# Daniel-Starr/pointcloudhookup

Measured on AMD Instinct MI355X. Metric: Mpts/s ground-filter+tower-cluster, 100 M-pt corridor; % HBM roofline on kNN, higher is better.
Workload: dtype f32 (filter) + f64 (distance predicate)

## Files before the change

pointcloudhookup_amd/csrc/pch_dbscan.hip:

```cpp
#include <assert.h>
#include "pch_prims.h"

namespace pch {

constexpr int DB_THREADS = 256;
constexpr int DB_WAVES   = DB_THREADS / 64;
constexpr int DB_ROWS    = 25;
constexpr int INT_BIG    = 0x7fffffff;
constexpr int DB_FEW_QUERIES = 24;
constexpr int DB_AHEAD = 3;
constexpr long long DB_LONG_TOT = 8192;
constexpr int DB_SEGS = 43;

struct DbGrid {
    float   ox, oy, oz;
    double  cell;
    double  inv_cell;
    double  eps2;
    float   eps2_lo, eps2_hi;
    int     bx, by, bz;
    int     mx, my, mz;
    int64_t chunk_size;
    const uint32_t* chunk_bad;
    const uint32_t* chunk_cells;
// ... 760 lines not shown
    int over = 0;
#pragma unroll
    for (int u = 0; u < CC_ITEMS; ++u) {
        const int c = c0 + u;
        v[u] = 0u;
        if (c < nchunks) {
            const int64_t lo = (int64_t)c * chunk_size;
            v[u] = ct_staged_cells(ncell, c, (n - lo) < chunk_size ? (n - lo) : chunk_size);
            over |= ovf[c] != 0u;
        }
        sum += v[u];
    }
    over = __syncthreads_or(over);
    const uint32_t incl = wave_scan_incl(sum);
    if (lane_id() == 63) wsum[wave_id()] = incl;
    __syncthreads();
    uint32_t run = incl - sum, total = 0;
    for (int w = 0; w < CC_THREADS / 64; ++w) { if (w < wave_id()) run += wsum[w]; total += wsum[w]; }
#pragma unroll
    for (int u = 0; u < CC_ITEMS; ++u) {
        if (c0 + u < nchunks) chunk_cells[c0 + u] = run;
        run += v[u];
    }
    if (tid == 0) {
        *route = over ? 1u : 0u;
        if (!over) {
            chunk_cells[nchunks] = total;
            cell_start[total] = (uint32_t)n;
            *ncells = total;
        }
    }
}

__global__ __launch_bounds__(DB_THREADS) void db_celltab_k(
    const uint32_t* __restrict__ route, DbStage st, const uint32_t* __restrict__ ovf,
    const uint32_t* __restrict__ chunk_cells, int64_t n, int64_t chunk_size, uint32_t* __restrict__ cid,
    uint32_t* __restrict__ cell_start, uint64_t* __restrict__ cell_key, int* __restrict__ cell_min,
    uint32_t* __restrict__ bits, uint64_t* __restrict__ keys_out) {
    const int64_t base = (int64_t)blockIdx.x * SCAN_TILE + (int64_t)threadIdx.x * DC_ITEMS;
    const bool fill = *route != 0u;
    if (!fill && base / DC_ITEMS < (n + 31) / 32) bits[base / DC_ITEMS] = 0u;
    if (base >= n) return;
    int64_t c = (uint32_t)base / (uint32_t)chunk_size;
    int64_t lo = c * chunk_size, end = lo + chunk_size < n ? lo + chunk_size : n;
    uint32_t nc = ct_staged_cells(st.ncell, c, end - lo), j = 0;
    for (uint32_t a = 1, b = nc; a < b;) {
        const uint32_t mid = a + (b - a) / 2;
        if (st.start[lo + mid] <= (uint32_t)base) { j = mid; a = mid + 1; } else b = mid;
    }
    int64_t next = j + 1 < nc ? (int64_t)st.start[lo + j + 1] : end;
    uint32_t cell0 = chunk_cells[c];
    bool skip = fill && ovf[c] != 0u;
    uint32_t cc[DC_ITEMS];
#pragma unroll
    for (int u = 0; u < DC_ITEMS; ++u) {
        const int64_t i = base + u;
        cc[u] = 0u;
        if (i >= n) continue;
        bool head = i == base && nc != 0u && (int64_t)st.start[lo + j] == i;
        if (i == end) {
            ++c; lo = end; end = lo + chunk_size < n ? lo + chunk_size : n;
            nc = ct_staged_cells(st.ncell, c, end - lo); j = 0;
            next = 1 < nc ? (int64_t)st.start[lo + 1] : end;
            cell0 = chunk_cells[c];
            skip = fill && ovf[c] != 0u;
            head = nc != 0u;
        } else if (i == next) {
            ++j;
            next = j + 1 < nc ? (int64_t)st.start[lo + j + 1] : end;
            head = true;
        }
        cc[u] = cell0 + j;
        if (fill) {
            if (!skip) keys_out[i] = st.key[lo + j];
        } else if (head) {
            cell_start[cc[u]] = (uint32_t)i;
            cell_key[cc[u]] = st.key[lo + j];
            cell_min[cc[u]] = (int)st.minrow[lo + j];
        }
    }
    if (fill) return;
    if (base + DC_ITEMS <= n) {
        uint4* o = reinterpret_cast<uint4*>(cid + base);
        o[0] = make_uint4(cc[0], cc[1], cc[2], cc[3]);
        o[1] = make_uint4(cc[4], cc[5], cc[6], cc[7]);
    } else {
#pragma unroll
        for (int u = 0; u < DC_ITEMS; ++u)
            if (base + u < n) cid[base + u] = cc[u];
    }
}

struct RowSet {
    int ca[DB_ROWS], cb[DB_ROWS];
};

template <typename K>
__device__ __forceinline__ int db_lower(const K* __restrict__ a, int m, K k) {
    int lo = 0, hi = m;
    while (lo < hi) { const int mid = (lo + hi) >> 1; if (a[mid] < k) lo = mid + 1; else hi = mid; }
    return lo;
}
struct DbRowAt { int xlo, xhi, ny, nz; };
__device__ __forceinline__ bool db_row_at(const DbGrid& g, uint64_t key, int row, DbRowAt& at) {
    const uint64_t cx = key & ((1ull << g.bx) - 1);
    const uint64_t cy = (key >> g.bx) & ((1ull << g.by) - 1);
    const uint64_t cz = (key >> (g.bx + g.by)) & ((1ull << g.bz) - 1);
    at.ny = (int)cy + DB_ROW_DY[row];
    at.nz = (int)cz + DB_ROW_DZ[row];
    at.xlo = (int)cx - 2 < 0 ? 0 : (int)cx - 2;
    at.xhi = (int)cx + 2 > g.mx ? g.mx : (int)cx + 2;
    return at.ny >= 0 && at.ny <= g.my && at.nz >= 0 && at.nz <= g.mz;
}
template <typename K>
__device__ __forceinline__ int2 db_run_in(const K* __restrict__ a, int n, K klo, K khi) {
    int2 v;
    v.x = db_lower(a, n, klo);
    K kk[5];
#pragma unroll
    for (int i = 0; i < 5; ++i) kk[i] = v.x + i < n ? a[v.x + i] : ~K(0);
    int cntx = 0;
#pragma unroll
    for (int i = 0; i < 5; ++i) cntx += kk[i] <= khi ? 1 : 0;
    v.y = v.x + cntx;
    return v;
// ... 11 lines not shown
                      db_pack(g, chunk, (uint64_t)at.nz, (uint64_t)at.ny, (uint64_t)at.xhi));
        v.x += c0;
        v.y += c0;
    }
    return v;
}

__device__ __forceinline__ void db_rows(const DbGrid& g, const uint64_t* __restrict__ cell_key, uint64_t key,
                                        RowSet* __restrict__ rs, const int2* __restrict__ rowtab, int cell) {
    const int l = lane_id();
    if (rowtab) {
        if (l < DB_ROWS) {
            const int2 v = rowtab[(int64_t)cell * DB_ROWS + l];
            rs->ca[l] = v.x;
            rs->cb[l] = v.y;
        }
        __builtin_amdgcn_wave_barrier();
        return;
    }
    if (l < DB_ROWS) {
        const int2 v = db_row_run(g, cell_key, key, l);
        rs->ca[l] = v.x;
        rs->cb[l] = v.y;
    }
    __builtin_amdgcn_wave_barrier();
}

__global__ __launch_bounds__(DB_THREADS) void db_rowtab_k(DbGrid g, const uint64_t* __restrict__ cell_key,
                                                          int m, int2* __restrict__ rowtab) {
    const int c = (blockIdx.x * DB_WAVES + wave_id()) * 2 + (lane_id() >> 5);
    const int l = lane_id() & 31;
    if (c >= m || l >= DB_ROWS) return;
    rowtab[(int64_t)c * DB_ROWS + l] = db_row_run(g, cell_key, cell_key[c], l);
}

template <bool COUNT, int AHEAD>
__device__ __forceinline__ int db_query_sweep(const DbGrid& g, const float4* __restrict__ pts, const float4 qp,
                                              int count, int r, uint32_t j0, const uint32_t* sa, const uint32_t* sb,
                                              unsigned long long& n_useful, unsigned long long& n_slots) {
    const int l = lane_id();
    while (r < DB_SEGS && count < g.min_samples) {
        const uint32_t pb = sb[r];
        if (j0 >= pb) { ++r; if (r < DB_SEGS) j0 = sa[r]; continue; }
        float4 P[AHEAD];
#pragma unroll
        for (int u = 0; u < AHEAD; ++u) {
            const uint32_t j = j0 + 64u * u + l;
            P[u] = pts[j < pb ? j : pb - 1];
        }
#pragma unroll
        for (int u = 0; u < AHEAD; ++u) {
            const uint32_t jb = j0 + 64u * u;
            const bool hit = jb + l < pb && db_within2(qp, P[u], g);
            count += (int)__popcll(__ballot(hit));
            if (COUNT && jb < pb) { n_useful += (pb - jb) < 64u ? (pb - jb) : 64u; n_slots += 64; }
        }
        j0 += 64u * AHEAD;
    }
    return count;
}

__device__ __forceinline__ void db_summary_none(float* __restrict__ cell_box, int* __restrict__ cell_min, int c) {
    const int l = lane_id();
    if (l < 6) cell_box[6 * (int64_t)c + l] = l < 3 ? INFINITY : -INFINITY;
    if (l == 0) cell_min[c] = INT_BIG;
}
// ... 869 lines not shown
    __syncthreads();

    int r = -1;
    if (tid < nc && ncore[tid] != 0) {
        r = uf_find(parent, tid);
        if (r != tid) atomicMin(&cmin[r], cmin[tid]);
    }
    __syncthreads();
    if (tid < nc) {
        const int64_t c = first + tid;
        root[c] = r < 0 ? -1 : first + r;
        comp_min[c] = r == tid ? cmin[tid] : INT_BIG;
        if (r == tid) {
            const uint32_t row = (uint32_t)cmin[tid];
            if ((int64_t)row < n) atomicOr(&flag[row >> 5], 1u << (row & 31u));
        }
    }
}

constexpr int DB_LAB_ROUNDS = 8;
constexpr int DB_LAB_TILE   = DB_THREADS * DB_LAB_ROUNDS;

__device__ __forceinline__ void db_box_flush(uint32_t* __restrict__ acc, int cur, uint32_t (&m)[6]) {
    const int l = lane_id();
    uint32_t v = 0;
#pragma unroll
    for (int a = 0; a < 6; ++a) {
        const uint32_t t = wave_reduce_max(m[a]);
        if (l == a) v = t;
        m[a] = 0u;
    }
    if (cur >= 0 && l < 6 && v) atomicMax(&acc[8 * (int64_t)cur + l], v);
}

__global__ __launch_bounds__(DB_THREADS) void db_label_k(const float4* __restrict__ pts,
                                                         const uint32_t* __restrict__ cid,
                                                         const uint8_t* __restrict__ core_s,
                                                         const int* __restrict__ root,
                                                         const int* __restrict__ comp_min,
                                                         const uint32_t* __restrict__ bits,
                                                         const uint32_t* __restrict__ rank, int64_t n,
                                                         const uint32_t* __restrict__ cell_start,
                                                         int* __restrict__ cell_label,
                                                         int32_t* __restrict__ labels,
                                                         uint8_t* __restrict__ core_out, int64_t chunk_size, int bpc,
                                                         int64_t nchunks, uint32_t* __restrict__ box_acc,
                                                         int32_t box_cap) {
    int64_t lo, hi;
    {
        const int64_t woff = (int64_t)wave_id() * (64 * DB_LAB_ROUNDS);
        if (bpc > 0) {
            const int64_t slot = blockIdx.x >> 3;
            const int64_t c = (slot / bpc) * 8 + (blockIdx.x & 7);
            const int64_t within = (slot % bpc) * DB_LAB_TILE + woff;
            lo = c * chunk_size + within;
            hi = (c < nchunks && within < chunk_size) ? (c + 1) * chunk_size : lo;
        } else {
            lo = (int64_t)blockIdx.x * DB_LAB_TILE + woff;
            hi = n;
        }
        if (hi > n) hi = n;
        if (hi > lo + 64 * DB_LAB_ROUNDS) hi = lo + 64 * DB_LAB_ROUNDS;
    }
    if (lo >= hi) return;
    const int l = lane_id();
    constexpr int R = DB_LAB_ROUNDS;
// ... 8 lines not shown
        c[u] = valid[u] ? cid[i] : 0u;
        p[u] = pts[valid[u] ? i : lo];
        is_core[u] = valid[u] && core_s[i] != 0;
    }
#pragma unroll
    for (int u = 0; u < R; ++u) {
        rt[u] = valid[u] ? root[c[u]] : -1;
        cs[u] = valid[u] ? cell_start[c[u]] : 0xFFFFFFFFu;
    }
#pragma unroll
    for (int u = 0; u < R; ++u) row[u] = rt[u] >= 0 ? (uint32_t)comp_min[rt[u]] : 0u;
#pragma unroll
    for (int u = 0; u < R; ++u) {
        rk[u] = rt[u] >= 0 ? rank[row[u] >> 5] : 0u;
        bw[u] = rt[u] >= 0 ? bits[row[u] >> 5] : 0u;
    }
#pragma unroll
    for (int u = 0; u < R; ++u) {
        const int64_t i = lo + u * 64 + l;
        lab[u] = rt[u] >= 0 ? (int)(rk[u] + (uint32_t)__popc(bw[u] & ((1u << (row[u] & 31u)) - 1u))) : INT_BIG;
        if (valid[u]) {
            const uint32_t o = __float_as_uint(p[u].w);
            labels[o] = is_core[u] ? lab[u] : -1;
            if (core_out) core_out[o] = is_core[u] ? 1 : 0;
            if (cs[u] == (uint32_t)i) cell_label[c[u]] = lab[u];
        }
    }
    if (!box_acc) return;
    int cur = -1;
    uint32_t m[6] = {0u, 0u, 0u, 0u, 0u, 0u};
#pragma unroll
    for (int u = 0; u < R; ++u) {
        const int mine = (is_core[u] && lab[u] != INT_BIG && lab[u] >= 0 && lab[u] < box_cap) ? lab[u] : -1;
        const uint32_t k[3] = {f32_ordered(p[u].x), f32_ordered(p[u].y), f32_ordered(p[u].z)};
        unsigned long long todo = __ballot(mine >= 0);
        while (todo) {
            const int L = __builtin_amdgcn_readlane(mine, (int)__builtin_ctzll(todo));
            const bool in = mine == L;
            todo &= ~__ballot(in);
            if (L != cur) {
                db_box_flush(box_acc, cur, m);
                cur = L;
            }
            if (in) {
#pragma unroll
                for (int a = 0; a < 3; ++a) {
                    m[a] = ~k[a] > m[a] ? ~k[a] : m[a];
                    m[3 + a] = k[a] > m[3 + a] ? k[a] : m[3 + a];
                }
            }
        }
    }
    db_box_flush(box_acc, cur, m);
}

constexpr int DB_BR = 3, DB_BROWS = 12;
struct DbCoreCells {
    int cell[DB_BR], label[DB_BR];
    bool dense[DB_BR];
    float box[DB_BR][6];
};

__device__ __forceinline__ void db_gather_core_cells(DbCoreCells& cc, const RowSet* __restrict__ rs, bool on,
                                                     const uint32_t* __restrict__ cell_start,
                                                     const uint32_t* __restrict__ cell_ncore,
                                                     const float* __restrict__ cell_box,
                                                     const int* __restrict__ cell_label) {
    const int l = lane_id();
#pragma unroll
    for (int rd = 0; rd < DB_BR; ++rd) {
        const int row = rd * DB_BROWS + l / 5, k = l % 5;
        cc.cell[rd] = -1; cc.label[rd] = INT_BIG; cc.dense[rd] = false;
#pragma unroll
        for (int a = 0; a < 6; ++a) cc.box[rd][a] = 0.0f;
        if (on && l < 5 * DB_BROWS && row < DB_ROWS) {
            const int B = rs->ca[row] + k;
            if (B < rs->cb[row]) {
                const uint32_t nb = cell_ncore[B];
                if (nb != 0) {
                    cc.cell[rd] = B;
                    cc.label[rd] = cell_label[B];
                    cc.dense[rd] = nb == cell_start[B + 1] - cell_start[B];
#pragma unroll
                    for (int a = 0; a < 6; ++a) cc.box[rd][a] = cell_box[6 * (int64_t)B + a];
                }
            }
// ... 9 lines not shown
    bool cand[DB_BR];
#pragma unroll
    for (int rd = 0; rd < DB_BR; ++rd) cand[rd] = cc.cell[rd] >= 0 && !(db_box_d2(qp, cc.box[rd]) > g.eps2);
    for (;;) {
        int mine = INT_BIG, sel = -1;
#pragma unroll
        for (int rd = 0; rd < DB_BR; ++rd)
            if (cand[rd] && cc.label[rd] < mine) { mine = cc.label[rd]; sel = rd; }
        const int lo = wave_reduce_min(mine);
        if (lo == INT_BIG) return INT_BIG;
        const int owner = (int)__builtin_ctzll(__ballot(mine == lo));
        int Bsel = -1;
        bool dsel = false;
#pragma unroll
        for (int rd = 0; rd < DB_BR; ++rd)
            if (sel == rd) { Bsel = cc.cell[rd]; dsel = cc.dense[rd]; }
        const int B = __builtin_amdgcn_readlane(Bsel, owner);
        const bool b_dense = __builtin_amdgcn_readlane((int)dsel, owner) != 0;
        const uint32_t bs = cell_start[B], be = cell_start[B + 1];
        for (uint32_t j0 = bs; j0 < be; j0 += 64) {
            const uint32_t j = j0 + l;
            bool hit = false;
            if (j < be && (b_dense || core_s[j])) hit = db_within2(qp, pts[j], g);
            if (__ballot(hit)) return lo;
        }
        if (l == owner) {
#pragma unroll
            for (int rd = 0; rd < DB_BR; ++rd)
                if (sel == rd) cand[rd] = false;
        }
    }
}

__global__ __launch_bounds__(DB_THREADS) void db_border_k(DbGrid g, const float4* __restrict__ pts,
                                                          const uint32_t* __restrict__ cell_start,
                                                          const uint64_t* __restrict__ cell_key, int m,
                                                          const int2* __restrict__ rowtab,
                                                          const uint8_t* __restrict__ core_s,
                                                          const uint32_t* __restrict__ cell_ncore,
                                                          const float* __restrict__ cell_box,
                                                          const int* __restrict__ cell_label,
                                                          int32_t* __restrict__ labels,
                                                          uint32_t* __restrict__ box_acc, int32_t box_cap) {
    __shared__ RowSet rows[DB_WAVES];
    const int A = blockIdx.x * DB_WAVES + wave_id();
    if (A >= m) return;
    const uint32_t as = cell_start[A], ae = cell_start[A + 1];
    if (cell_ncore[A] == (ae - as)) return;
    const int l = lane_id();
    RowSet* rs = &rows[wave_id()];
    db_rows(g, cell_key, cell_key[A], rs, rowtab, A);
    int any = 0;
    if (l < DB_ROWS)
        for (int B = rs->ca[l]; B < rs->cb[l]; ++B) any |= (cell_ncore[B] != 0);
    if (!__ballot(any != 0)) return;
    DbCoreCells cc;
    db_gather_core_cells(cc, rs, true, cell_start, cell_ncore, cell_box, cell_label);
    for (uint32_t q = as; q < ae; ++q) {
        if (core_s[q]) continue;
        const float4 qp = pts[q];
        const int best = db_border_label(g, qp, cc, pts, cell_start, core_s);
        if (l == 0 && best != INT_BIG) labels[__float_as_uint(qp.w)] = best;
        if (box_acc && best != INT_BIG && best >= 0 && best < box_cap && l < 6) {
            const float v = l % 3 == 0 ? qp.x : (l % 3 == 1 ? qp.y : qp.z);
            const uint32_t k = f32_ordered(v);
            atomicMax(&box_acc[8 * (int64_t)best + l], l < 3 ? ~k : k);
        }
    }
}

struct DbQuery {
    const float* xyz; int64_t nq;
    float sx, sy, sz;
    const int32_t* chunk;
    int64_t nchunks;
};
constexpr uint32_t DQ_OUT   = 0x80000000u;
#ifndef PCH_DQ_PIECE
#define PCH_DQ_PIECE 64
#endif
constexpr int      DQ_PIECE = PCH_DQ_PIECE;

__device__ __forceinline__ float4 dq_point(const DbQuery& Q, int64_t i) {
    float4 q;
    q.x = Q.xyz[3 * i + 0] - Q.sx; q.y = Q.xyz[3 * i + 1] - Q.sy; q.z = Q.xyz[3 * i + 2] - Q.sz; q.w = 0.0f;
    return q;
}

__global__ __launch_bounds__(DB_THREADS) void dq_keys_k(DbQuery Q, DbGrid g, uint64_t* __restrict__ keys,
                                                        uint32_t* __restrict__ vals) {
    const int64_t i = (int64_t)blockIdx.x * DB_THREADS + threadIdx.x;
    if (i >= Q.nq) return;
    const float4 q = dq_point(Q, i);
    const int64_t c = Q.chunk ? (int64_t)Q.chunk[i] : 0;
    bool ok = c >= 0 && c < Q.nchunks;
// ... 458 lines not shown
                fprintf(stderr, "chunksort phase %d: %.2f us\n", q, (double)(long long)(t[q] - t[q - 1]) / 100.0);
            fprintf(stderr, "chunksort tiles: rank %.2f us, offsets %.2f us, scatter %.2f us\n", (double)t[8] / 100.0,
                    (double)t[9] / 100.0, (double)t[10] / 100.0);
        }
#endif
        ks = w.k1;
        return PCH_OK;
    }
    PCH_HIP_TRY(hipMemsetAsync(w.chunk_bad, 0, sizeof(uint32_t) * (size_t)(nchunks + 1), s));
    if (compressed) {
        PCH_LAUNCH("db_keys_comp", db_keys_comp_k, dim3(gn), dim3(DB_THREADS), 0, s, w.comp, n, g, w.k0, w.v0);
    } else {
        PCH_LAUNCH("db_chunkbad", db_chunkbad_k, dim3(db_stride_blocks(n)), dim3(DB_THREADS), 0, s, r.xyz, n,
                   r.chunk_size, w.chunk_bad);
        PCH_LAUNCH("db_keys", db_keys_k, dim3(gn), dim3(DB_THREADS), 0, s, r.xyz, n, g, w.chunk_bad, w.k0, w.v0,
                   &w.meta->status);
    }
    PCH_TRY(radix_sort_pairs(w.k0, w.v0, w.k1, w.v1, n, nbits, w.radix_ws, s));
    const bool in1 = radix_sort_result_buffer(nbits) == 1;
    ks = in1 ? w.k1 : w.k0;
    PCH_LAUNCH("db_gather", db_gather_k, dim3(gn), dim3(DB_THREADS), 0, s, r.xyz, ks, in1 ? w.v1 : w.v0, n, w.pts);
    return PCH_OK;
}

static int db_cells_core(const DbRun& r, const DbGrid& g, int cellbits, const uint64_t* ks, bool staged,
                         bool count_pairs, DbCells& c) {
    const DbWs& w = r.w; const hipStream_t s = r.s; const int64_t n = r.n;
    const int64_t ntile = ceil_div(n, (int64_t)SCAN_TILE);
    DbMeta back;
    constexpr size_t peek_bytes = offsetof(DbMeta, pad) + sizeof(uint32_t) - offsetof(DbMeta, status);
    back.pad[0] = 1u;
    if (staged) {
        PCH_TRY(peek_enqueue(&w.meta->status, peek_bytes, s));
        PCH_LAUNCH("db_celltab", db_celltab_k, dim3((unsigned)ntile), dim3(DB_THREADS), 0, s, w.cell_route, w.stage,
                   w.chunk_ovf, w.chunk_cells, n, r.chunk_size, w.cid, w.cell_start, w.cell_key, w.cell_min, w.bits, w.k1);
        PCH_TRY(peek_wait(&back.status, peek_bytes));
    }
    if (back.pad[0] != 0u) {
        PCH_LAUNCH("db_heads", db_heads_k, dim3((unsigned)ntile), dim3(DB_THREADS), 0, s, ks, n, w.scan_ws);
        PCH_TRY(scan_tile_sums_u32(w.scan_ws, ntile, &w.meta->ncells, s));
        PCH_TRY(peek_enqueue(&w.meta->status, 2 * sizeof(uint32_t), s));
        PCH_LAUNCH("db_cells", db_cells_k, dim3((unsigned)ntile), dim3(DB_THREADS), 0, s, ks, w.scan_ws, n, cellbits,
                   r.nchunks, w.cid, w.cell_start, w.cell_key, w.chunk_cells, w.cell_acc);
        PCH_TRY(peek_wait(&back.status, 2 * sizeof(uint32_t)));
    }
    if (back.status != 0) {
        set_error("finite coordinates outside the supplied bounding box");
        return PCH_ERR_ARG;
    }
    const int m = (int)back.ncells;
    const unsigned gc = (unsigned)ceil_div(m, DB_WAVES);
    c = {g, w.pts, w.cell_start, w.cell_key, m, m <= w.rowtab_cells ? w.rowtab : nullptr, w.core_s, w.cell_ncore,
         w.cell_box, staged && back.pad[0] == 0u};
    if (c.rowtab)
        PCH_LAUNCH("db_rowtab", db_rowtab_k, dim3((unsigned)ceil_div(m, 2 * DB_WAVES)), dim3(DB_THREADS), 0, s, g,
                   w.cell_key, m, w.rowtab);
    float* const sum_box = c.chunk_union ? w.cell_box : nullptr;
    int* const sum_min = c.chunk_union ? w.cell_min : nullptr;
    if (count_pairs) {
        PCH_HIP_TRY(hipMemsetAsync(w.core_stats, 0, 4 * sizeof(unsigned long long), s));
        PCH_LAUNCH("db_core_counting", db_core_k<true>, dim3(gc), dim3(DB_THREADS), 0, s, DB_GRID_ARGS(c), w.core_s,
                   w.cell_ncore, sum_box, sum_min, w.core_stats);
    } else {
        PCH_LAUNCH("db_core", db_core_k<false>, dim3(gc), dim3(DB_THREADS), 0, s, DB_GRID_ARGS(c), w.core_s,
                   w.cell_ncore, sum_box, sum_min, nullptr);
    }
    if (!c.chunk_union) {
        PCH_LAUNCH("db_cellstats", db_cellstats_k, dim3((unsigned)ceil_div(n, (int64_t)DB_WAVES * 64 * DB_CS_ROUNDS)),
                   dim3(DB_THREADS), 0, s, w.pts, w.cid, w.core_s, n, w.cell_acc, w.bits, ceil_div(n, 32));
        PCH_LAUNCH("db_cellfin", db_cellfin_k, dim3((unsigned)ceil_div(m, DB_THREADS)), dim3(DB_THREADS), 0, s,
                   w.cell_acc, m, w.cell_box, w.cell_min, w.parent, w.comp_min);
    }
    return PCH_OK;
}

static int db_union(const DbRun& r, const DbCells& c) {
    const DbWs& w = r.w; const hipStream_t s = r.s; const int m = c.m;
    const unsigned gc = (unsigned)ceil_div(m, DB_WAVES);
    if (c.chunk_union) {
        PCH_LAUNCH("db_chunkunion", db_chunkunion_k, dim3((unsigned)r.nchunks), dim3(CU_THREADS), 0, s, c.g, c.pts,
                   c.cell_start, c.cell_key, m, c.core_s, c.cell_ncore, c.cell_box, w.cell_min, w.root, w.comp_min,
                   w.bits, r.n);
        return PCH_OK;
    }
    if (c.rowtab)
        PCH_LAUNCH("db_union_pairs", db_union_pairs_k, dim3((unsigned)ceil_div(4 * (int64_t)m, DB_THREADS)),
                   dim3(DB_THREADS), 0, s, DB_CELL_ARGS(c), w.parent, w.face_todo);
    PCH_LAUNCH("db_union0", db_union_face_k, dim3(gc), dim3(DB_THREADS), 0, s, DB_CELL_ARGS(c), w.parent,
               c.rowtab ? (const uint8_t*)w.face_todo : nullptr);
    PCH_LAUNCH("db_flatten", db_flatten_k, dim3((unsigned)ceil_div(m, DB_THREADS)), dim3(DB_THREADS), 0, s,
               w.parent, m);
    PCH_LAUNCH("db_union1", db_union_k, dim3(gc), dim3(DB_THREADS), 0, s, DB_CELL_ARGS(c), w.parent);
    PCH_LAUNCH("db_compmin", db_compmin_k, dim3((unsigned)ceil_div(m, DB_THREADS)), dim3(DB_THREADS), 0, s,
               w.cell_min, w.cell_ncore, m, w.parent, w.root, w.comp_min);
    return PCH_OK;
}

static int db_labels(const DbRun& r, const DbCells& c, int32_t* k_host, DbBoxOut* boxes) {
    const DbWs& w = r.w; const hipStream_t s = r.s; const int64_t n = r.n, nchunks = r.nchunks; const int m = c.m;
    const int64_t nw = ceil_div(n, 32);
    static_assert(DB_CS_ROUNDS * 64 * DB_WAVES / DB_THREADS <= 32, "db_cellstats_k's grid has a thread per bitmap word");
    if (!c.chunk_union)
        PCH_LAUNCH("db_mark", db_mark_k, dim3((unsigned)ceil_div(m, DB_THREADS)), dim3(DB_THREADS), 0, s,
                   w.root, w.comp_min, m, w.bits);
    if (scan1_pays(nw)) PCH_TRY(scan1_exclusive_popc_u32(w.bits, w.wrank, nw, w.scan1_b, &w.meta->nclusters, s));
    else PCH_TRY(scan_exclusive_popc_u32(w.bits, w.wrank, nw, w.scan_ws, &w.meta->nclusters, s));
    uint32_t* box_acc = (boxes && boxes->acc && boxes->cap > 0) ? boxes->acc : nullptr;
    const int32_t box_cap = box_acc ? boxes->cap : 0;
    PCH_LAUNCH("db_prelabel", db_prelabel_k, dim3((unsigned)(box_acc ? ceil_div(8 * (int64_t)box_cap, 256) : 1)),
               dim3(256), 0, s, &w.meta->nclusters, r.out_nclusters, box_acc, 8 * (int64_t)box_cap);
    if (k_host) PCH_TRY(peek_enqueue(r.out_nclusters, sizeof(int32_t), s));
    const int bpc = nchunks >= 16 ? (int)ceil_div(r.chunk_size, DB_LAB_TILE) : 0;
    const unsigned gl = bpc > 0 ? (unsigned)(8 * ceil_div(nchunks, 8) * bpc) : (unsigned)ceil_div(n, DB_LAB_TILE);
    PCH_LAUNCH("db_label", db_label_k, dim3(gl), dim3(DB_THREADS), 0, s, w.pts, w.cid, w.core_s, w.root, w.comp_min,
               w.bits, w.wrank, n, w.cell_start, w.cell_label, r.labels, r.core, r.chunk_size, bpc, nchunks, box_acc,
               box_cap);
    PCH_LAUNCH("db_border", db_border_k, dim3((unsigned)ceil_div(m, DB_WAVES)), dim3(DB_THREADS), 0, s,
               DB_CELL_ARGS(c), w.cell_label, r.labels, box_acc, box_cap);
    if (box_acc) boxes->done = true;
    if (k_host) {
        PCH_TRY(peek_wait(k_host, sizeof(int32_t)));
        if (*k_host < 0) {
            set_error("stage C: a device-side look-back wait ran out of its budget; outputs are undefined");
            return PCH_ERR_TIMEOUT;
        }
    }
    return PCH_OK;
}

}

using namespace pch;

extern "C" int pch_first_nonfinite_row_f32(const float* xyz, int64_t n, int64_t* out_row, void* stream) {
    PCH_DEVICE_GUARD(out_row);
    hipStream_t s = (hipStream_t)stream;
    PCH_REQUIRE(n >= 0 && out_row && (n == 0 || xyz), "bad argument");
    PCH_HIP_TRY(hipMemsetAsync(out_row, 0xFF, sizeof(int64_t), s));
    if (n == 0) return PCH_OK;
    PCH_LAUNCH("db_first_bad", db_first_bad_k, dim3(db_stride_blocks(n)), dim3(DB_THREADS), 0, s, xyz, n,
               reinterpret_cast<unsigned long long*>(out_row));
    return PCH_OK;
}

extern "C" void pch_dbscan_set_sort_mode(int mode) {
    __atomic_store_n(&g_sort_mode, (mode == 1 || mode == 2) ? mode : 0, __ATOMIC_RELAXED);
}

extern "C" size_t pch_dbscan_ws_bytes(int64_t n) {
    if (n < 0) return 0;
    Arena a;
// ... 74 lines not shown
    PCH_HIP_TRY(hipStreamSynchronize((hipStream_t)stream));
    return PCH_OK;
}

extern "C" int pch_dbscan_strip_pairs_i32(int64_t n, float x_lo, float x_hi, int32_t cap, int32_t* out_pairs,
                                          int32_t* out_count, void* ws, size_t ws_bytes, void* stream) {
    PCH_DEVICE_GUARD(out_count);
    hipStream_t s = (hipStream_t)stream;
    PCH_REQUIRE(n >= 0 && cap >= 0 && out_count && (cap == 0 || out_pairs), "bad argument");
    PCH_HIP_TRY(hipMemsetAsync(out_count, 0, sizeof(int32_t), s));
    if (n == 0 || !(x_lo < x_hi)) return PCH_OK;
    DbWs w;
    PCH_TRY(db_continue(__func__, n, ws, ws_bytes, w));
    const int m = g_last.c.m;
    PCH_LAUNCH("db_strip_pairs", db_strip_pairs_k, dim3((unsigned)ceil_div(m, DB_WAVES)), dim3(DB_THREADS), 0, s,
               w.pts, w.cell_start, w.core_s, w.cell_ncore, w.cell_box, w.cell_label, m, x_lo, x_hi, cap, out_pairs,
               out_count);
    return PCH_OK;
}

extern "C" int pch_dbscan_relabel_i32(const int32_t* map, int32_t nmap, int64_t n, int32_t* labels, void* ws,
                                      size_t ws_bytes, void* stream) {
    PCH_DEVICE_GUARD(labels);
    hipStream_t s = (hipStream_t)stream;
    PCH_REQUIRE(n >= 0 && nmap >= 0 && (nmap == 0 || map) && (n == 0 || labels), "bad argument");
    if (n == 0) return PCH_OK;
    DbWs w;
    PCH_TRY(db_continue(__func__, n, ws, ws_bytes, w));
    const DbCells& c = g_last.c;
    PCH_LAUNCH("db_remap_points", db_remap_points_k, dim3((unsigned)ceil_div(n, DB_THREADS)), dim3(DB_THREADS), 0, s,
               w.pts, w.core_s, n, map, nmap, labels);
    PCH_LAUNCH("db_remap_cells", db_remap_cells_k, dim3((unsigned)ceil_div(c.m, DB_THREADS)), dim3(DB_THREADS), 0, s,
               w.cell_label, w.cell_ncore, c.m, map, nmap);
    PCH_LAUNCH("db_border", db_border_k, dim3((unsigned)ceil_div(c.m, DB_WAVES)), dim3(DB_THREADS), 0, s,
               DB_CELL_ARGS(c), w.cell_label, labels, nullptr, 0);
    return PCH_OK;
}

struct DqWs { uint64_t *k0, *k1; uint32_t *v0, *v1, *flag, *piece_start, *radix_ws, *scan_ws, *npieces; };
static void dq_plan(Arena& a, int64_t nq, DqWs& w) {
    const int64_t nn = nq > 0 ? nq : 1;
    w.npieces = a.take<uint32_t>(64);
    w.k0 = a.take<uint64_t>(nn);
    w.k1 = a.take<uint64_t>(nn);
    w.v0 = a.take<uint32_t>(nn);
    w.v1 = a.take<uint32_t>(nn);
    w.flag = a.take<uint32_t>(nn + 8);
    w.piece_start = a.take<uint32_t>(nn + 8);
    w.radix_ws = a.take<uint32_t>(radix_ws_u32(nn));
    w.scan_ws = a.take<uint32_t>(scan_ws_u32(nn));
}

extern "C" size_t pch_dbscan_assign_ws_bytes(int64_t nq) {
    if (nq < 0) return 0;
    Arena a;
    DqWs w;
    dq_plan(a, nq, w);
    return a.off;
}

extern "C" int pch_dbscan_assign_f32(const float* query, int64_t nq, const float* sub3_host, const int32_t* query_chunk,
                                     int64_t n, int32_t* out_labels, void* qws, size_t qws_bytes, void* ws,
                                     size_t ws_bytes, void* stream) {
    PCH_DEVICE_GUARD(out_labels ? (const void*)out_labels : (const void*)ws);
    hipStream_t s = (hipStream_t)stream;
    PCH_REQUIRE(nq >= 0 && nq < (int64_t(1) << 31), "nq out of range [0, 2^31)");
    PCH_REQUIRE(n >= 0, "bad argument");
    if (nq == 0) return PCH_OK;
// ... 47 lines not shown
```

profiles/summarize.py:

```python
#!/usr/bin/env python3
import collections
import csv
import glob
import json
import os
import sys

tag, stats_dir, fetch_dir, write_dir, points = sys.argv[1:6]
kind = sys.argv[6] if len(sys.argv) > 6 else "corridor"
frame = sys.argv[7] if len(sys.argv) > 7 else "offset"
sq_dirs = sys.argv[8:]
here = os.path.dirname(os.path.abspath(__file__))


def short(name):
    name = name.replace("void ", "")
    return name.split("(")[0].replace("pch::", "")


rows = list(csv.DictReader(open(glob.glob(os.path.join(stats_dir, "**/*kernel_stats.csv"), recursive=True)[0])))
ours = [r for r in rows if "pch::" in r["Name"]]
with open(os.path.join(here, f"{tag}_kernel_stats.csv"), "w") as f:
    f.write("kernel,calls,avg_us,min_us,max_us,total_ms,percent_of_all_gpu_time\n")
    for r in sorted(ours, key=lambda r: -float(r["TotalDurationNs"])):
        f.write(f"{short(r['Name'])},{r['Calls']},{float(r['AverageNs']) / 1e3:.2f},{float(r['MinNs']) / 1e3:.2f},"
                f"{float(r['MaxNs']) / 1e3:.2f},{float(r['TotalDurationNs']) / 1e6:.3f},{r['Percentage']}\n")


def pmc(d, counter):
    acc = collections.defaultdict(list)
    for r in csv.DictReader(open(glob.glob(os.path.join(d, "**/*counter_collection.csv"), recursive=True)[0])):
        if r["Counter_Name"] == counter and "pch::" in r["Kernel_Name"]:
            acc[short(r["Kernel_Name"])].append(float(r["Counter_Value"]))
    return acc


fetch, write = pmc(fetch_dir, "FETCH_SIZE"), pmc(write_dir, "WRITE_SIZE")
steps_in_stats = 6
steps_in_pmc = 3
names = {"ms_summary_k": "mean_summary", "ms_walk_k": "mean_walk", "ms_level2_k": "mean_level2",
         "db_core_k": "db_core", "db_core_k<false>": "db_core", "db_core_k<true>": "db_core_counting",
         "db_union_pairs_k": "db_union_pairs", "db_mark_k": "db_mark", "sel_bracket_k": "sel_bracket",
         "sg_hist_k": "seg_hist", "sg_scatter_k": "seg_scatter", "db_union_k": "db_union", "db_border_k": "db_border",
         "gf_compact_k<0>": "gf_compact", "gf_compact_k<1>": "gf_compact_fb", "db_chunksort_k": "db_chunksort", "db_cellscatter_k": "db_cellscatter",
         "db_cellscatter_k<true>": "db_cellscatter", "db_cellscatter_k<false>": "db_cellscatter",
         "db_chunkcells_k": "db_chunkcells", "db_celltab_k": "db_celltab",
         "sel_hist_k<0, 1, true>": "sel_hist0",
         "sel_hist_k<1, 1, true>": "sel_hist1", "sel_hist_k<2, 1, true>": "sel_hist2", "rs_scatter_k": "radix_scatter",
         "rs_hist_k": "radix_hist", "db_gather_k": "db_gather", "db_keys_k": "db_keys",
         "sg_stats_k": "seg_stats", "db_label_k": "db_label", "db_cellbox_k": "db_cellbox",
         "db_union_face_k": "db_union0", "db_rowtab_k": "db_rowtab", "db_cellstats_k": "db_cellstats",
         "db_cells_k": "db_cells", "ms_sample_k": "mean_sample", "ms_prefix_k": "mean_prefix",
         "scan1_k<false>": "scan1", "scan1_k<true>": "scan1_popc", "db_prelabel_k": "db_prelabel",
         "sl_hist_k": "seg_hist", "sl_scatter_k": "seg_scatter", "sl_offsets_k": "seg_offsets",
         "vx_finish_k": "voxel_finish", "vx_scatter_k": "voxel_scatter", "vx_scatter_lds_k": "voxel_scatter",
         "vx_tilehist_k": "voxel_tilehist", "vx_minmax_k": "voxel_minmax", "vx_split_k": "voxel_split",
         "vx_binscan_k": "voxel_binscan", "db_chunkunion_k": "db_chunkunion"}
sys.path.insert(0, here)
from stamp import csrc_sha
traffic = {"points": int(points), "kind": kind, "frame": frame, "source": tag, "csrc_sha": csrc_sha(),
           "unit": "bytes per launch (2*FETCH_SIZE + WRITE_SIZE, KiB->B)", "kernels": {}}
with open(os.path.join(here, f"{tag}_pmc_traffic.csv"), "w") as f:
    f.write("kernel,launches,fetch_bytes_raw_per_launch,fetch_bytes_x2_per_launch,write_bytes_per_launch\n")
    for k in sorted(set(fetch) | set(write), key=lambda k: -sum(fetch.get(k, [0]))):
        fl, wl = fetch.get(k, []), write.get(k, [])
        fb = 1024 * sum(fl) / max(len(fl), 1)
        wb = 1024 * sum(wl) / max(len(wl), 1)
        f.write(f"{k},{max(len(fl), len(wl))},{fb:.0f},{2 * fb:.0f},{wb:.0f}\n")
        if k in names:
            traffic["kernels"][names[k]] = int(2 * fb + wb)
traffic["launches_per_step"] = round(sum(int(r["Calls"]) for r in ours) / steps_in_stats, 2)
traffic["kernel_ms_per_step"] = round(sum(float(r["TotalDurationNs"]) for r in ours) / 1e6 / steps_in_stats, 4)
tot = 0.0
for k in set(fetch) | set(write):
    tot += 1024 * (2 * sum(fetch.get(k, [])) + sum(write.get(k, [])))
traffic["step_bytes"] = int(tot / steps_in_pmc)
traffic["avg_us"] = {names.get(short(r["Name"]), short(r["Name"])): round(float(r["AverageNs"]) / 1e3, 2) for r in ours}
if sq_dirs:
    sq = collections.defaultdict(dict)
    for d in sq_dirs:
        files = glob.glob(os.path.join(d, "**/*counter_collection.csv"), recursive=True)
        if not files:
            continue
        acc = collections.defaultdict(lambda: collections.defaultdict(list))
        for r in csv.DictReader(open(files[0])):
            if "pch::" in r["Kernel_Name"]:
                acc[short(r["Kernel_Name"])][r["Counter_Name"]].append(float(r["Counter_Value"]))
        for k, cs in acc.items():
            for c, v in cs.items():
                sq[k][c] = sum(v) / max(len(v), 1)
# ... 22 lines not shown
```

Baseline: 69850.

## Restructure DBSCAN cell-table build per chunk and label chunk-union path by hashed cell lookup

The cell table kernel is now launched one block per chunk instead of per point tile. It writes per-cell start, key and min directly from staged data, and also builds the neighbour row table in LDS, so the separate rowtab kernel is skipped on the chunk-union path. The per-point cell id write is gone. On that path, labels come from a new kernel that hashes each point's cell key into a shared-memory table of per-chunk cell labels, with a cell-level prelabel kernel in front. Border handling takes over labelling of mixed cells, which drops the cid array traffic but adds per-point key recomputation, hash probing and more complex control flow.

```diff
diff --git a/pointcloudhookup_amd/csrc/pch_dbscan.hip b/pointcloudhookup_amd/csrc/pch_dbscan.hip
--- a/pointcloudhookup_amd/csrc/pch_dbscan.hip
+++ b/pointcloudhookup_amd/csrc/pch_dbscan.hip
@@ -816,65 +816,6 @@
     }
 }
 
-__global__ __launch_bounds__(DB_THREADS) void db_celltab_k(
-    const uint32_t* __restrict__ route, DbStage st, const uint32_t* __restrict__ ovf,
-    const uint32_t* __restrict__ chunk_cells, int64_t n, int64_t chunk_size, uint32_t* __restrict__ cid,
-    uint32_t* __restrict__ cell_start, uint64_t* __restrict__ cell_key, int* __restrict__ cell_min,
-    uint32_t* __restrict__ bits, uint64_t* __restrict__ keys_out) {
-    const int64_t base = (int64_t)blockIdx.x * SCAN_TILE + (int64_t)threadIdx.x * DC_ITEMS;
-    const bool fill = *route != 0u;
-    if (!fill && base / DC_ITEMS < (n + 31) / 32) bits[base / DC_ITEMS] = 0u;
-    if (base >= n) return;
-    int64_t c = (uint32_t)base / (uint32_t)chunk_size;
-    int64_t lo = c * chunk_size, end = lo + chunk_size < n ? lo + chunk_size : n;
-    uint32_t nc = ct_staged_cells(st.ncell, c, end - lo), j = 0;
-    for (uint32_t a = 1, b = nc; a < b;) {
-        const uint32_t mid = a + (b - a) / 2;
-        if (st.start[lo + mid] <= (uint32_t)base) { j = mid; a = mid + 1; } else b = mid;
-    }
-    int64_t next = j + 1 < nc ? (int64_t)st.start[lo + j + 1] : end;
-    uint32_t cell0 = chunk_cells[c];
-    bool skip = fill && ovf[c] != 0u;
-    uint32_t cc[DC_ITEMS];
-#pragma unroll
-    for (int u = 0; u < DC_ITEMS; ++u) {
-        const int64_t i = base + u;
-        cc[u] = 0u;
-        if (i >= n) continue;
-        bool head = i == base && nc != 0u && (int64_t)st.start[lo + j] == i;
-        if (i == end) {
-            ++c; lo = end; end = lo + chunk_size < n ? lo + chunk_size : n;
-            nc = ct_staged_cells(st.ncell, c, end - lo); j = 0;
-            next = 1 < nc ? (int64_t)st.start[lo + 1] : end;
-            cell0 = chunk_cells[c];
-            skip = fill && ovf[c] != 0u;
-            head = nc != 0u;
-        } else if (i == next) {
-            ++j;
-            next = j + 1 < nc ? (int64_t)st.start[lo + j + 1] : end;
-            head = true;
-        }
-        cc[u] = cell0 + j;
-        if (fill) {
-            if (!skip) keys_out[i] = st.key[lo + j];
-        } else if (head) {
-            cell_start[cc[u]] = (uint32_t)i;
-            cell_key[cc[u]] = st.key[lo + j];
-            cell_min[cc[u]] = (int)st.minrow[lo + j];
-        }
-    }
-    if (fill) return;
-    if (base + DC_ITEMS <= n) {
-        uint4* o = reinterpret_cast<uint4*>(cid + base);
-        o[0] = make_uint4(cc[0], cc[1], cc[2], cc[3]);
-        o[1] = make_uint4(cc[4], cc[5], cc[6], cc[7]);
-    } else {
-#pragma unroll
-        for (int u = 0; u < DC_ITEMS; ++u)
-            if (base + u < n) cid[base + u] = cc[u];
-    }
-}
-
 struct RowSet {
     int ca[DB_ROWS], cb[DB_ROWS];
 };
@@ -952,6 +893,57 @@
     const int l = lane_id() & 31;
     if (c >= m || l >= DB_ROWS) return;
     rowtab[(int64_t)c * DB_ROWS + l] = db_row_run(g, cell_key, cell_key[c], l);
+}
+
+__global__ __launch_bounds__(CS_THREADS) void db_celltab_k(
+    const uint32_t* __restrict__ route, DbStage st, const uint32_t* __restrict__ ovf, DbGrid g, int64_t n,
+    uint32_t* __restrict__ cell_start, uint64_t* __restrict__ cell_key, int* __restrict__ cell_min,
+    uint32_t* __restrict__ bits, int2* __restrict__ rowtab, int64_t rowtab_cells, uint64_t* __restrict__ keys_out) {
+    __shared__ uint32_t key[CT_CELLS];
+    const int tid = threadIdx.x, l = lane_id();
+    const int64_t c = blockIdx.x, lo = c * g.chunk_size;
+    const int64_t end = lo + g.chunk_size < n ? lo + g.chunk_size : n;
+    const bool fill = *route != 0u;
+    if (fill && ovf[c] != 0u) return;
+    int nc = (int)ct_staged_cells(st.ncell, c, end - lo);
+    nc = nc > CT_CELLS ? CT_CELLS : nc;
+    if (fill) {
+        for (int j = wave_id(); j < nc; j += CS_WAVES) {
+            int64_t a = st.start[lo + j], b = j + 1 < nc ? (int64_t)st.start[lo + j + 1] : end;
+            a = a < lo ? lo : a;
+            b = b > end ? end : b;
+            const uint64_t k = st.key[lo + j];
+            for (int64_t i = a + l; i < b; i += 64) keys_out[i] = k;
+        }
+        return;
+    }
+    const int64_t cell0 = g.chunk_cells[c];
+    if (cell0 + nc > n) return;
+    for (int64_t wd = (lo >> 5) + tid; wd <= ((end - 1) >> 5); wd += CS_THREADS) bits[wd] = 0u;
+    if (tid < nc) {
+        const uint64_t k = st.key[lo + tid];
+        cell_start[cell0 + tid] = st.start[lo + tid];
+        cell_key[cell0 + tid] = k;
+        cell_min[cell0 + tid] = (int)st.minrow[lo + tid];
+        const int sh = g.bx + g.by + g.bz;
+        key[tid] = (uint32_t)k & ((1u << sh) - 1u);
+    }
+    if (!rowtab) return;
+    __syncthreads();
+    for (int t = tid; t < 32 * nc; t += CS_THREADS) {
+        const int j = t >> 5, row = t & 31;
+        if (row >= DB_ROWS || cell0 + j >= rowtab_cells) continue;
+        int2 v;
+        v.x = 0; v.y = 0;
+        DbRowAt at;
+        if (db_row_at(g, key[j], row, at)) {
+            v = db_run_in(key, nc, (uint32_t)db_pack(g, 0, (uint64_t)at.nz, (uint64_t)at.ny, (uint64_t)at.xlo),
+                          (uint32_t)db_pack(g, 0, (uint64_t)at.nz, (uint64_t)at.ny, (uint64_t)at.xhi));
+            v.x += (int)cell0;
+            v.y += (int)cell0;
+        }
+        rowtab[(cell0 + j) * DB_ROWS + row] = v;
+    }
 }
 
 template <bool COUNT, int AHEAD>
@@ -1887,6 +1879,27 @@
     }
     if (cur >= 0 && l < 6 && v) atomicMax(&acc[8 * (int64_t)cur + l], v);
 }
+__device__ __forceinline__ void db_box_round(uint32_t* __restrict__ acc, int& cur, uint32_t (&m)[6], int mine, float x,
+                                             float y, float z) {
+    const uint32_t k[3] = {f32_ordered(x), f32_ordered(y), f32_ordered(z)};
+    unsigned long long todo = __ballot(mine >= 0);
+    while (todo) {
+        const int L = __builtin_amdgcn_readlane(mine, (int)__builtin_ctzll(todo));
+        const bool in = mine == L;
+        todo &= ~__ballot(in);
+        if (L != cur) {
+            db_box_flush(acc, cur, m);
+            cur = L;
+        }
+        if (in) {
+#pragma unroll
+            for (int a = 0; a < 3; ++a) {
+                m[a] = ~k[a] > m[a] ? ~k[a] : m[a];
+                m[3 + a] = k[a] > m[3 + a] ? k[a] : m[3 + a];
+            }
+        }
+    }
+}
 
 __global__ __launch_bounds__(DB_THREADS) void db_label_k(const float4* __restrict__ pts,
                                                          const uint32_t* __restrict__ cid,
@@ -1961,26 +1974,136 @@
 #pragma unroll
     for (int u = 0; u < R; ++u) {
         const int mine = (is_core[u] && lab[u] != INT_BIG && lab[u] >= 0 && lab[u] < box_cap) ? lab[u] : -1;
-        const uint32_t k[3] = {f32_ordered(p[u].x), f32_ordered(p[u].y), f32_ordered(p[u].z)};
-        unsigned long long todo = __ballot(mine >= 0);
-        while (todo) {
-            const int L = __builtin_amdgcn_readlane(mine, (int)__builtin_ctzll(todo));
-            const bool in = mine == L;
-            todo &= ~__ballot(in);
-            if (L != cur) {
-                db_box_flush(box_acc, cur, m);
-                cur = L;
+        db_box_round(box_acc, cur, m, mine, p[u].x, p[u].y, p[u].z);
+    }
+    db_box_flush(box_acc, cur, m);
+}
+
+__global__ void db_prelabel_cells_k(const uint32_t* __restrict__ total, int32_t* __restrict__ out_nclusters,
+                                    uint32_t* __restrict__ box_acc, int64_t box_words,
+                                    const int* __restrict__ root, const int* __restrict__ comp_min,
+                                    const uint32_t* __restrict__ bits, const uint32_t* __restrict__ rank, int m,
+                                    int* __restrict__ cell_label) {
+    if (threadIdx.x == 0 && blockIdx.x == 0) *out_nclusters = (int32_t)*total;
+    const int64_t i = (int64_t)blockIdx.x * blockDim.x + threadIdx.x;
+    if (box_acc && i < box_words) box_acc[i] = 0u;
+    if (i >= m) return;
+    const int rt = root[i];
+    int lab = INT_BIG;
+    if (rt >= 0) {
+        const uint32_t row = (uint32_t)comp_min[rt];
+        lab = (int)(rank[row >> 5] + (uint32_t)__popc(bits[row >> 5] & ((1u << (row & 31u)) - 1u)));
+    }
+    cell_label[i] = lab;
+}
+
+constexpr int DB_FL_NONE = -0x7fffffff - 1;
+constexpr int FL_SLOTS = 2 * CT_CELLS;
+__device__ __forceinline__ uint32_t fl_hash(uint32_t k) { return (k * 0x9E3779B1u) >> 21; }
+static_assert(FL_SLOTS == 1 << 11, "fl_hash yields 11 bits");
+
+__global__ __launch_bounds__(DB_THREADS) void db_filelabel_k(const float* __restrict__ xyz, int64_t n, DbGrid g,
+                                                             const uint32_t* __restrict__ cell_start,
+                                                             const uint64_t* __restrict__ cell_key, int m,
+                                                             const uint32_t* __restrict__ cell_ncore,
+                                                             const int* __restrict__ cell_label,
+                                                             int32_t* __restrict__ labels,
+                                                             uint8_t* __restrict__ core_out, int bpc, int64_t nchunks,
+                                                             uint32_t* __restrict__ box_acc, int32_t box_cap) {
+    __shared__ uint2 tab[FL_SLOTS];
+    const int tid = threadIdx.x;
+    const int64_t slot = blockIdx.x >> 3;
+    const int64_t c = (slot / bpc) * 8 + (blockIdx.x & 7);
+    const int64_t within = (slot % bpc) * DB_LAB_TILE;
+    if (c >= nchunks || within >= g.chunk_size) return;
+    const int64_t t0 = c * g.chunk_size + within;
+    int64_t t1 = (c + 1) * g.chunk_size < n ? (c + 1) * g.chunk_size : n;
+    if (t1 > t0 + DB_LAB_TILE) t1 = t0 + DB_LAB_TILE;
+    if (t0 >= t1) return;
+    constexpr int R = DB_LAB_ROUNDS;
+    const Row3* __restrict__ rows = reinterpret_cast<const Row3*>(xyz);
+    Row3 q[R];
+    uint32_t k[R];
+    int lab[R];
+#pragma unroll
+    for (int u = 0; u < R; ++u) {
+        const int64_t i = t0 + u * DB_THREADS + tid;
+        q[u] = rows[i < t1 ? i : t0];
+    }
+    if (g.chunk_bad[c]) {
+        for (int64_t i = t0 + tid; i < t1; i += DB_THREADS) {
+            labels[i] = -1;
+            if (core_out) core_out[i] = 0;
+        }
+        return;
+    }
+    int first = (int)g.chunk_cells[c], nc = (int)g.chunk_cells[c + 1] - first;
+    first = first < 0 ? 0 : (first > m ? m : first);
+    nc = nc < 0 ? 0 : (nc > CT_CELLS ? CT_CELLS : nc);
+    nc = nc > m - first ? m - first : nc;
+    const int sh = g.bx + g.by + g.bz;
+    for (int j = tid; j < FL_SLOTS; j += DB_THREADS) tab[j].x = CT_EMPTY;
+    __syncthreads();
+    for (int j = tid; j < nc; j += DB_THREADS) {
+        const int64_t A = first + j;
+        const uint32_t key = (uint32_t)cell_key[A] & ((1u << sh) - 1u);
+        const int label = cell_ncore[A] == cell_start[A + 1] - cell_start[A] ? cell_label[A] : DB_FL_NONE;
+        uint32_t h = fl_hash(key);
+        for (int p = 0; p < FL_SLOTS; ++p, h = (h + 1u) & (FL_SLOTS - 1))
+            if (atomicCAS(&tab[h].x, CT_EMPTY, key) == CT_EMPTY) { tab[h].y = (uint32_t)label; break; }
+    }
+#pragma unroll
+    for (int u = 0; u < R; ++u) {
+        bool ok;
+        k[u] = cs_cell_key(g, q[u].x, q[u].y, q[u].z, ok);
+    }
+    __syncthreads();
+#pragma unroll
+    for (int u = 0; u < R; ++u) {
+        const int64_t i = t0 + u * DB_THREADS + tid;
+        lab[u] = DB_FL_NONE;
+        if (i < t1) {
+            uint32_t h = fl_hash(k[u]);
+            for (int p = 0; p < FL_SLOTS; ++p, h = (h + 1u) & (FL_SLOTS - 1)) {
+                const uint2 e = tab[h];
+                if (e.x == k[u]) { lab[u] = (int)e.y; break; }
+                if (e.x == CT_EMPTY) break;
             }
+        }
+        if (lab[u] != DB_FL_NONE) {
+            labels[i] = lab[u];
+            if (core_out) core_out[i] = 1;
+        }
+    }
+    if (!box_acc) return;
+    unsigned long long todo[R];
+#pragma unroll
+    for (int u = 0; u < R; ++u) {
+        if (!(lab[u] != DB_FL_NONE && lab[u] != INT_BIG && lab[u] >= 0 && lab[u] < box_cap)) lab[u] = -1;
+        todo[u] = __ballot(lab[u] >= 0);
+    }
+    for (;;) {
+        int L = -1;
+#pragma unroll
+        for (int u = 0; u < R; ++u)
+            if (L < 0 && todo[u]) L = __builtin_amdgcn_readlane(lab[u], (int)__builtin_ctzll(todo[u]));
+        if (L < 0) break;
+        uint32_t mm[6] = {0u, 0u, 0u, 0u, 0u, 0u};
+#pragma unroll
+        for (int u = 0; u < R; ++u) {
+            const bool in = lab[u] == L;
+            todo[u] &= ~__ballot(in);
             if (in) {
+                const uint32_t kk[3] = {f32_ordered(q[u].x), f32_ordered(q[u].y), f32_ordered(q[u].z)};
 #pragma unroll
                 for (int a = 0; a < 3; ++a) {
-                    m[a] = ~k[a] > m[a] ? ~k[a] : m[a];
-                    m[3 + a] = k[a] > m[3 + a] ? k[a] : m[3 + a];
+                    mm[a] = ~kk[a] > mm[a] ? ~kk[a] : mm[a];
+                    mm[3 + a] = kk[a] > mm[3 + a] ? kk[a] : mm[3 + a];
                 }
             }
         }
-    }
-    db_box_flush(box_acc, cur, m);
+        db_box_flush(box_acc, L, mm);
+    }
 }
 
 constexpr int DB_BR = 3, DB_BROWS = 12;
@@ -2056,6 +2179,7 @@
     }
 }
 
+template <bool OWN>
 __global__ __launch_bounds__(DB_THREADS) void db_border_k(DbGrid g, const float4* __restrict__ pts,
                                                           const uint32_t* __restrict__ cell_start,
                                                           const uint64_t* __restrict__ cell_key, int m,
@@ -2065,26 +2189,48 @@
                                                           const float* __restrict__ cell_box,
                                                           const int* __restrict__ cell_label,
                                                           int32_t* __restrict__ labels,
-                                                          uint32_t* __restrict__ box_acc, int32_t box_cap) {
+                                                          uint32_t* __restrict__ box_acc, int32_t box_cap,
+                                                          uint8_t* __restrict__ core_out) {
     __shared__ RowSet rows[DB_WAVES];
     const int A = blockIdx.x * DB_WAVES + wave_id();
     if (A >= m) return;
     const uint32_t as = cell_start[A], ae = cell_start[A + 1];
-    if (cell_ncore[A] == (ae - as)) return;
+    const uint32_t ncoreA = cell_ncore[A];
+    if (ncoreA == (ae - as)) return;
     const int l = lane_id();
+    if constexpr (OWN) {
+        const int sh = g.bx + g.by + g.bz;
+        if (g.chunk_bad[sh < 64 ? (cell_key[A] >> sh) : 0]) return;
+        const int labA = cell_label[A];
+        for (uint32_t q = as + l; q < ae; q += 64) {
+            const bool is_core = core_s[q] != 0;
+            const uint32_t o = __float_as_uint(pts[q].w);
+            if (is_core) labels[o] = labA;
+            if (core_out) core_out[o] = is_core ? 1 : 0;
+        }
+        if (box_acc && ncoreA != 0 && labA != INT_BIG && labA >= 0 && labA < box_cap && l < 6) {
+            const uint32_t k = f32_ordered(cell_box[6 * (int64_t)A + l]);
+            atomicMax(&box_acc[8 * (int64_t)labA + l], l < 3 ? ~k : k);
+        }
+    }
     RowSet* rs = &rows[wave_id()];
     db_rows(g, cell_key, cell_key[A], rs, rowtab, A);
     int any = 0;
     if (l < DB_ROWS)
         for (int B = rs->ca[l]; B < rs->cb[l]; ++B) any |= (cell_ncore[B] != 0);
-    if (!__ballot(any != 0)) return;
+    if (!__ballot(any != 0)) {
+        if constexpr (OWN)
+            for (uint32_t q = as + l; q < ae; q += 64)
+                if (!core_s[q]) labels[__float_as_uint(pts[q].w)] = -1;
+        return;
+    }
     DbCoreCells cc;
     db_gather_core_cells(cc, rs, true, cell_start, cell_ncore, cell_box, cell_label);
     for (uint32_t q = as; q < ae; ++q) {
         if (core_s[q]) continue;
         const float4 qp = pts[q];
         const int best = db_border_label(g, qp, cc, pts, cell_start, core_s);
-        if (l == 0 && best != INT_BIG) labels[__float_as_uint(qp.w)] = best;
+        if (l == 0 && (OWN || best != INT_BIG)) labels[__float_as_uint(qp.w)] = best != INT_BIG ? best : -1;
         if (box_acc && best != INT_BIG && best >= 0 && best < box_cap && l < 6) {
             const float v = l % 3 == 0 ? qp.x : (l % 3 == 1 ? qp.y : qp.z);
             const uint32_t k = f32_ordered(v);
@@ -2609,8 +2755,8 @@
     back.pad[0] = 1u;
     if (staged) {
         PCH_TRY(peek_enqueue(&w.meta->status, peek_bytes, s));
-        PCH_LAUNCH("db_celltab", db_celltab_k, dim3((unsigned)ntile), dim3(DB_THREADS), 0, s, w.cell_route, w.stage,
-                   w.chunk_ovf, w.chunk_cells, n, r.chunk_size, w.cid, w.cell_start, w.cell_key, w.cell_min, w.bits, w.k1);
+        PCH_LAUNCH("db_celltab", db_celltab_k, dim3((unsigned)r.nchunks), dim3(CS_THREADS), 0, s, w.cell_route, w.stage,
+                   w.chunk_ovf, g, n, w.cell_start, w.cell_key, w.cell_min, w.bits, w.rowtab, w.rowtab_cells, w.k1);
         PCH_TRY(peek_wait(&back.status, peek_bytes));
     }
     if (back.pad[0] != 0u) {
@@ -2629,7 +2775,7 @@
     const unsigned gc = (unsigned)ceil_div(m, DB_WAVES);
     c = {g, w.pts, w.cell_start, w.cell_key, m, m <= w.rowtab_cells ? w.rowtab : nullptr, w.core_s, w.cell_ncore,
          w.cell_box, staged && back.pad[0] == 0u};
-    if (c.rowtab)
+    if (c.rowtab && !c.chunk_union)
         PCH_LAUNCH("db_rowtab", db_rowtab_k, dim3((unsigned)ceil_div(m, 2 * DB_WAVES)), dim3(DB_THREADS), 0, s, g,
                    w.cell_key, m, w.rowtab);
     float* const sum_box = c.chunk_union ? w.cell_box : nullptr;
@@ -2684,16 +2830,29 @@
     else PCH_TRY(scan_exclusive_popc_u32(w.bits, w.wrank, nw, w.scan_ws, &w.meta->nclusters, s));
     uint32_t* box_acc = (boxes && boxes->acc && boxes->cap > 0) ? boxes->acc : nullptr;
     const int32_t box_cap = box_acc ? boxes->cap : 0;
-    PCH_LAUNCH("db_prelabel", db_prelabel_k, dim3((unsigned)(box_acc ? ceil_div(8 * (int64_t)box_cap, 256) : 1)),
-               dim3(256), 0, s, &w.meta->nclusters, r.out_nclusters, box_acc, 8 * (int64_t)box_cap);
+    const int64_t box_words = box_acc ? 8 * (int64_t)box_cap : 0;
+    if (c.chunk_union)
+        PCH_LAUNCH("db_prelabel", db_prelabel_cells_k, dim3((unsigned)std::max<int64_t>(ceil_div(std::max<int64_t>(
+                   box_words, m), 256), 1)), dim3(256), 0, s, &w.meta->nclusters, r.out_nclusters, box_acc, box_words,
+                   w.root, w.comp_min, w.bits, w.wrank, m, w.cell_label);
+    else
+        PCH_LAUNCH("db_prelabel", db_prelabel_k, dim3((unsigned)std::max<int64_t>(ceil_div(box_words, 256), 1)),
+                   dim3(256), 0, s, &w.meta->nclusters, r.out_nclusters, box_acc, box_words);
     if (k_host) PCH_TRY(peek_enqueue(r.out_nclusters, sizeof(int32_t), s));
-    const int bpc = nchunks >= 16 ? (int)ceil_div(r.chunk_size, DB_LAB_TILE) : 0;
+    const int bpc = (nchunks >= 16 || c.chunk_union) ? (int)ceil_div(r.chunk_size, DB_LAB_TILE) : 0;
     const unsigned gl = bpc > 0 ? (unsigned)(8 * ceil_div(nchunks, 8) * bpc) : (unsigned)ceil_div(n, DB_LAB_TILE);
-    PCH_LAUNCH("db_label", db_label_k, dim3(gl), dim3(DB_THREADS), 0, s, w.pts, w.cid, w.core_s, w.root, w.comp_min,
-               w.bits, w.wrank, n, w.cell_start, w.cell_label, r.labels, r.core, r.chunk_size, bpc, nchunks, box_acc,
-               box_cap);
-    PCH_LAUNCH("db_border", db_border_k, dim3((unsigned)ceil_div(m, DB_WAVES)), dim3(DB_THREADS), 0, s,
-               DB_CELL_ARGS(c), w.cell_label, r.labels, box_acc, box_cap);
+    if (c.chunk_union) {
+        PCH_LAUNCH("db_label", db_filelabel_k, dim3(gl), dim3(DB_THREADS), 0, s, r.xyz, n, c.g, c.cell_start, c.cell_key,
+                   m, c.cell_ncore, w.cell_label, r.labels, r.core, bpc, nchunks, box_acc, box_cap);
+        PCH_LAUNCH("db_border", db_border_k<true>, dim3((unsigned)ceil_div(m, DB_WAVES)), dim3(DB_THREADS), 0, s,
+                   DB_CELL_ARGS(c), w.cell_label, r.labels, box_acc, box_cap, r.core);
+    } else {
+        PCH_LAUNCH("db_label", db_label_k, dim3(gl), dim3(DB_THREADS), 0, s, w.pts, w.cid, w.core_s, w.root, w.comp_min,
+                   w.bits, w.wrank, n, w.cell_start, w.cell_label, r.labels, r.core, r.chunk_size, bpc, nchunks, box_acc,
+                   box_cap);
+        PCH_LAUNCH("db_border", db_border_k<false>, dim3((unsigned)ceil_div(m, DB_WAVES)), dim3(DB_THREADS), 0, s,
+                   DB_CELL_ARGS(c), w.cell_label, r.labels, box_acc, box_cap, nullptr);
+    }
     if (box_acc) boxes->done = true;
     if (k_host) {
         PCH_TRY(peek_wait(k_host, sizeof(int32_t)));
@@ -2834,8 +2993,8 @@
                w.pts, w.core_s, n, map, nmap, labels);
     PCH_LAUNCH("db_remap_cells", db_remap_cells_k, dim3((unsigned)ceil_div(c.m, DB_THREADS)), dim3(DB_THREADS), 0, s,
                w.cell_label, w.cell_ncore, c.m, map, nmap);
-    PCH_LAUNCH("db_border", db_border_k, dim3((unsigned)ceil_div(c.m, DB_WAVES)), dim3(DB_THREADS), 0, s,
-               DB_CELL_ARGS(c), w.cell_label, labels, nullptr, 0);
+    PCH_LAUNCH("db_border", db_border_k<false>, dim3((unsigned)ceil_div(c.m, DB_WAVES)), dim3(DB_THREADS), 0, s,
+               DB_CELL_ARGS(c), w.cell_label, labels, nullptr, 0, nullptr);
     return PCH_OK;
 }
 
diff --git a/profiles/summarize.py b/profiles/summarize.py
--- a/profiles/summarize.py
+++ b/profiles/summarize.py
@@ -55,7 +55,8 @@
          "sl_hist_k": "seg_hist", "sl_scatter_k": "seg_scatter", "sl_offsets_k": "seg_offsets",
          "vx_finish_k": "voxel_finish", "vx_scatter_k": "voxel_scatter", "vx_scatter_lds_k": "voxel_scatter",
          "vx_tilehist_k": "voxel_tilehist", "vx_minmax_k": "voxel_minmax", "vx_split_k": "voxel_split",
-         "vx_binscan_k": "voxel_binscan", "db_chunkunion_k": "db_chunkunion"}
+         "vx_binscan_k": "voxel_binscan", "db_chunkunion_k": "db_chunkunion", "db_filelabel_k": "db_label",
+         "db_prelabel_cells_k": "db_prelabel", "db_border_k<true>": "db_border", "db_border_k<false>": "db_border"}
 sys.path.insert(0, here)
 from stamp import csrc_sha
 traffic = {"points": int(points), "kind": kind, "frame": frame, "source": tag, "csrc_sha": csrc_sha(),
```

Result: faster. 71660, median of 6 (+2.6%).
